# zerohd4869/MM-DFN

Hardware: AMD Instinct MI355X
Metric: utterances/sec (fwd+bwd), IEMOCAP-shaped batch (higher is better)
Workload: dtype f32; 1 GPU; cfg2 (BASELINE configs[1]): B=16 dialogues/GPU, L=110, dims 100/100/512, 2 GCN layers, P=2, dropout 0.50; utterances_per_gpu=1760, parallelism=dp1

## Files before the change

### include/mmdfn_hip.h

```cpp
#ifndef MMDFN_HIP_H
#define MMDFN_HIP_H

#include <stdint.h>

#ifdef __cplusplus
extern "C" {
#endif

int64_t mmdfn_riders_bytes(void);

int mmdfn_abi_version(void);

int mmdfn_propagate(const float* tiles, const float* cross, const float* H, float* out,
                    const int32_t* dia_len, const int32_t* row_start, const int64_t* tile_base,
                    int B, int M, int N, int d, int ldh, int ldo, int max_len, int transpose,
                    void* stream);

int mmdfn_tile_outer(const float* X, const float* Y, float* dtiles, float* dcross,
                     const int32_t* dia_len, const int32_t* row_start, const int64_t* tile_base,
                     int B, int M, int N, int d, int ldx, int ldy, int max_len, int accumulate,
                     void* stream);

int mmdfn_adj_build(const float* feats, float* unit, float* norm, float* cosg, float* cdot,
                    float* rdeg, float* tiles, float* cross,
// ... 52 lines not shown
int mmdfn_keep_flags_stage(float* out, int64_t n, float keep, void* state, void* riders, void* stream);
int mmdfn_keep_flags_flush(void* riders, void* stream);
int mmdfn_gru_seq_fwd_takes_flags(int ngroups, const int* rows);
int64_t mmdfn_colsum_workspace(int H);
int mmdfn_colsum(const float* A, int64_t R, int H, int lda, float* out, float* workspace, void* stream);
int mmdfn_colsum_partial(const float* A, int64_t R, int H, int lda, float* workspace, void* stream);
int mmdfn_party_combine(int Mn, const float* const* base, const float* E, const int32_t* rank,
                        const int64_t* flat_idx, float* out, const float* weights,
                        int L, int B, int P, int N, int H, void* stream);
int mmdfn_party_combine_bwd(int Mn, const float* dout, const int32_t* rank, const int64_t* flat_idx,
                            float* const* dbase, float* dE, const float* weights,
                            int L, int B, int P, int N, int H, void* stream);
int mmdfn_party_combine_bwd_dst(int Mn, const float* dout, const int32_t* rank, const int64_t* inv, float* const* dbase,
                                float* dE, const float* weights, int L, int B, int P, int N, int H, void* stream);


int mmdfn_mask_scale(int ngroups, const float* const* x, const float* const* mask, float* const* out,
                     const int64_t* n, float scale, void* stream);

int mmdfn_linear(const float* X, const float* W, const float* bias, float* Y, int R, int K, int N,
                 int ldx, int ldy, int act, int accumulate, void* stream);
int mmdfn_linear2(const float* X, const float* W, const float* W2, int N1, const float* bias, const float* bias2,
                  float* Y, int R, int K, int N, int ldx, int ldy, int act, int accumulate, void* stream);

int64_t mmdfn_weight_planes_workspace(int N, int K);
int mmdfn_cut_weight_planes(int n, const float* const* w1, const float* const* w2, const int* n1, const int* ld,
                            const int* N, const int* K, const int* mode, void* const* planes, void* stream);
int mmdfn_linear_planes(const float* X, const void* planes, const float* bias, const float* bias2, int n1, float* Y, int R,
                        int K, int N, int ldx, int ldy, int act, int accumulate, void* stream);
int mmdfn_linear_planes_group(int n, const float* const* X, const void* const* planes, const float* const* bias,
                              const float* const* bias2, const int* n1, float* const* Y, const int* R, const int* K,
                              const int* N, const int* ldx, const int* ldy, int act, int accumulate,
                              const float* const* mask, float mask_scale, void* stream);

int mmdfn_linear_group_supported(int R, int K, int N);
int mmdfn_linear_group(int n, const float* const* X, const float* const* W, const float* const* W2, const int* N1,
                       const float* const* bias, const float* const* bias2, float* const* Y, const int* R,
                       const int* K, const int* N, const int* ldx, const int* ldw, const int* ldy,
                       const int* kmajor, const int* accumulate, int act, void* stream);
int mmdfn_linear_group_addend(int n, const float* const* X, const float* const* W, const float* const* W2, const int* N1,
                              const float* const* bias, const float* const* bias2, float* const* Y, const float* const* Z,
                              const int* ldz, const int* R, const int* K, const int* N, const int* ldx, const int* ldw,
                              const int* ldy, const int* kmajor, const int* accumulate, int act, void* stream);

int mmdfn_softmax_scale_fwd(const float* z, const float* c, float* att, float* out, int R, int W, void* stream);
int mmdfn_softmax_scale_bwd(const float* att, const float* c, const float* dout, float* dz, float* dc, int R, int W,
                            void* stream);
int mmdfn_mfn_mem_fwd(const float* u, const float* v1, const float* v2, const float* mem, float* out, float* saved,
                      int64_t n, void* stream);
int mmdfn_mfn_mem_bwd(const float* saved, const float* mem, const float* dout, float* du, float* dv1, float* dv2,
                      float* dmem, int64_t n, void* stream);
int mmdfn_gated_pair_fwd(const float* xm, const float* xn, const float* w, const float* b, const float* pm,
                         const float* pn, float* out, float* zs, int R, int D, int C, void* stream);
int mmdfn_gated_pair_bwd(const float* xm, const float* xn, const float* w, const float* pm, const float* pn,
                         const float* zs, const float* dout, float* dxm, float* dxn, float* dpm, float* dpn,
                         float* dpre, int R, int D, int C, void* stream);
int mmdfn_rowscale_colsum(const float* s, const float* xm, const float* xn, float* out, int R, int D, void* stream);

int mmdfn_gemm_tn_splits(int R, int M, int N);
int mmdfn_gemm_tn(const float* A, const float* B, float* C, float* colsum, float* workspace,
                  int R, int M, int N, int lda, int ldb, int ldc, int splits, void* stream);

int64_t mmdfn_gemm_tn_grouped_workspace(int n, const int* R, const int* M, const int* N);
int mmdfn_gemm_tn_grouped(int n, const float* const* A, const float* const* B, float* const* C, float* const* colsum,
                          const int* R, const int* M, const int* N, const int* lda, const int* ldb, const int* ldc,
                          const int* bshift, float* workspace, void* stream);
// ... 87 lines not shown
```

### mm_dfn_amd/_hip.py

```python
import ctypes
import os

import torch

from . import build as _build

_P = ctypes.c_void_p
_I = ctypes.c_int
_F = ctypes.c_float
_L = ctypes.c_int64

SIGNATURES = {
    "mmdfn_abi_version": [],
    "mmdfn_propagate": [_P, _P, _P, _P, _P, _P, _P, _I, _I, _I, _I, _I, _I, _I, _I, _P],
    "mmdfn_tile_outer": [_P, _P, _P, _P, _P, _P, _P, _I, _I, _I, _I, _I, _I, _I, _I, _P],
    "mmdfn_adj_build": [_P] * 8 + [_P, _P, _P] + [_I] * 5 + [_F, _P],
    "mmdfn_adj_build_bwd": [_P] * 16 + [_P, _P, _P] + [_I] * 5 + [_F, _P],
    "mmdfn_riders_bytes": [],
    "mmdfn_gru_seq_fwd": [_I, _P, _P, _P, _P, _P, _P, _P, _I, _P, _P],
    "mmdfn_gru_seq_bwd": [_I, _P, _P, _P, _P, _P, _P, _P, _P, _I, _P, _P],
    "mmdfn_gru_seq_fwd_seg": [_I, _P, _P, _P, _P, _P, _P, _P, _I, _P, _P, _P, _P, _P, _P],
    "mmdfn_gru_seq_bwd_seg": [_I, _P, _P, _P, _P, _P, _P, _P, _P, _I, _P, _P, _P, _P, _P, _P, _P],
    "mmdfn_gru_tab_reduce": [_P, _P, _P, _P, _I, _I, _I, _I, _P],
    "mmdfn_lstm_pointwise_fwd": [_P, _P, _P, _P, _L, _I, _P],
    "mmdfn_lstm_pointwise_bwd": [_P, _P, _P, _P, _P, _P, _P, _L, _I, _P],
    "mmdfn_gcnii_combine_fwd": [_P, _P, _P, _P, _P, _F, _F, _L, _I, _P],
    "mmdfn_gcnii_combine_bwd": [_P, _P, _P, _P, _P, _P, _F, _F, _L, _I, _P],
    "mmdfn_gcn_input_fwd": [_P] * 8 + [_I] * 4 + [_F, _P],
    "mmdfn_gcn_input_bwd": [_P] * 9 + [_I] * 4 + [_F, _P],
    "mmdfn_lstm_gate_fwd": [_P] * 10 + [_I] * 2 + [_P],
    "mmdfn_lstm_gate_fwd_ld": [_P] * 10 + [_I] * 3 + [_P],
    "mmdfn_lstm_gate_fwd_pre": [_P] * 10 + [_I] * 3 + [_P, _P],
    "mmdfn_lstm_gate_planes_workspace": [_I],
    "mmdfn_lstm_gate_cut_weights": [_P, _P, _P, _I, _P],
    "mmdfn_lstm_gate_takes_planes": [_I, _I],
    "mmdfn_lstm_gate_bwd": [_P] * 13 + [_I] * 4 + [_P],
    "mmdfn_gcnii_layer_fwd": [_P] * 7 + [_F, _F, _I, _I, _I, _F, _P],
    "mmdfn_prop_layer_fwd": [_P, _P, _P, _I, _P, _P, _P, _I, _I, _I, _I, _P, _P, _P, _P, _P, _P, _P, _F, _F, _I, _I, _F, _P],
    "mmdfn_gcnii_layer_bwd": [_P] * 6 + [_F, _F, _I, _I, _I, _I, _P],
    "mmdfn_gcnii_layer_bwd_ld": [_P] * 6 + [_F, _F, _I, _I, _I, _I, _I, _P],
    "mmdfn_linear": [_P, _P, _P, _P, _I, _I, _I, _I, _I, _I, _I, _P],
    "mmdfn_linear2": [_P, _P, _P, _I, _P, _P, _P, _I, _I, _I, _I, _I, _I, _I, _P],
    "mmdfn_weight_planes_workspace": [_I, _I],
    "mmdfn_cut_weight_planes": [_I, _P, _P, _P, _P, _P, _P, _P, _P, _P],
    "mmdfn_linear_planes": [_P, _P, _P, _P, _I, _P, _I, _I, _I, _I, _I, _I, _I, _P],
    "mmdfn_linear_planes_group": [_I, _P, _P, _P, _P, _P, _P, _P, _P, _P, _P, _P, _I, _I, _P, _F, _P],
    "mmdfn_linear_group_supported": [_I, _I, _I],
    "mmdfn_linear_group": [_I] + [_P] * 15 + [_I, _P],
    "mmdfn_linear_group_addend": [_I] + [_P] * 17 + [_I, _P],
    "mmdfn_softmax_scale_fwd": [_P, _P, _P, _P, _I, _I, _P],
    "mmdfn_softmax_scale_bwd": [_P, _P, _P, _P, _P, _I, _I, _P],
    "mmdfn_mfn_mem_fwd": [_P] * 6 + [_L, _P],
    "mmdfn_mfn_mem_bwd": [_P] * 7 + [_L, _P],
    "mmdfn_gated_pair_fwd": [_P] * 8 + [_I, _I, _I, _P],
    "mmdfn_gated_pair_bwd": [_P] * 12 + [_I, _I, _I, _P],
    "mmdfn_rowscale_colsum": [_P, _P, _P, _P, _I, _I, _P],
    "mmdfn_gemm_tn_splits": [_I, _I, _I],
    "mmdfn_gemm_tn": [_P, _P, _P, _P, _P, _I, _I, _I, _I, _I, _I, _I, _P],
    "mmdfn_gemm_tn_grouped_workspace": [_I, _P, _P, _P],
    "mmdfn_gemm_tn_grouped": [_I, _P, _P, _P, _P, _P, _P, _P, _P, _P, _P, _P, _P, _P],
    "mmdfn_gemm_tn_batch_workspace": [_I, _P, _P, _I, _P, _P],
    "mmdfn_gemm_tn_batch": [_I, _P, _P, _P, _P, _P, _P, _P, _I, _P, _P, _P, _P, _P, _P, _P, _P, _P, _P],
    "mmdfn_wgrad_riders_stage": [_I, _P, _P, _P, _P, _P, _P, _P, _I, _P, _P, _P, _P, _P, _P, _P, _P, _P, _P],
    "mmdfn_wgrad_riders_staged": [_P],
    "mmdfn_wgrad_riders_flush": [_P, _P],
    "mmdfn_wgrad_riders_drain": [_P, _P, _I],
    "mmdfn_gru_seq_bwd_idle_cus": [_I, _P],
    "mmdfn_gru_seq_bwd_step_ns": [_I, _P],
    "mmdfn_gemm_tn_batch_ext": [_I, _P, _P, _P, _P, _P, _P, _P, _I, _P, _P, _P, _P, _P, _P, _P, _P,
                                _I, _P, _P, _P, _P, _P, _P, _P, _P, _P, _P, _P],
    "mmdfn_head_bwd_groups": [],
    "mmdfn_head_bwd_partial": [_P, _P, _P, _P, _P, _P, _P, _L, _I, _I, _I, _I, _I, _F, _P],
    "mmdfn_colsum_partial": [_P, _L, _I, _I, _P, _P],
    "mmdfn_head_fwd": [_P, _P, _P, _P, _P, _L, _I, _I, _I, _I, _F, _P],
    "mmdfn_head_bwd_workspace": [_I, _I],
    "mmdfn_head_bwd": [_P] * 9 + [_L, _I, _I, _I, _I, _I, _F, _P],
    "mmdfn_focal_loss_fwd": [_P, _P, _P, _P, _P, _L, _I, _F, _I, _P],
    "mmdfn_focal_loss_bwd": [_P, _P, _P, _P, _L, _I, _P],
    "mmdfn_focal_loss_fwd_grad": [_P, _P, _P, _P, _P, _P, _L, _I, _F, _I, _P],
    "mmdfn_focal_loss_fwd_ignore": [_P, _P, _P, _P, _P, _P, _L, _I, _F, _I, _L, _P],
    "mmdfn_focal_loss_bwd_ignore": [_P, _P, _P, _P, _P, _L, _I, _L, _P],
    "mmdfn_adam_step": [_P, _P, _P, _P, _L, _F, _F, _F, _F, _F, _I, _P],
    "mmdfn_party_gather": [_I, _P, _P, _P, _P, _P, _I, _I, _I, _I, _P],
    "mmdfn_party_gather_bwd": [_I, _P, _P, _P, _P, _I, _I, _I, _I, _P],
    "mmdfn_party_gather_bwd_colsum": [_I, _P, _P, _P, _P, _I, _I, _I, _I, _P, _P],
    "mmdfn_party_combine": [_I, _P, _P, _P, _P, _P, _P, _I, _I, _I, _I, _I, _P],
    "mmdfn_party_combine_bwd": [_I, _P, _P, _P, _P, _P, _P, _I, _I, _I, _I, _I, _P],
    "mmdfn_party_combine_bwd_dst": [_I, _P, _P, _P, _P, _P, _P, _I, _I, _I, _I, _I, _P],
    "mmdfn_mask_scale": [_I, _P, _P, _P, _P, _F, _P],
    "mmdfn_keep_flags": [_P, _L, _F, _P, _P],
    "mmdfn_keep_flags_stage": [_P, _L, _F, _P, _P, _P],
    "mmdfn_keep_flags_flush": [_P, _P],
    "mmdfn_gru_seq_fwd_takes_flags": [_I, _P],
    "mmdfn_colsum_workspace": [_I],
    "mmdfn_colsum": [_P, _L, _I, _I, _P, _P, _P],
}

ABI_VERSION = 18


class HipLibraryError(RuntimeError):
    pass


_libs = {}
_tuning = os.environ.get("MMDFN_TUNING_LIB", "0") == "1"


def set_tuning(flag):
    global _tuning
    prev, _tuning = _tuning, bool(flag)
    return prev


def lib():
    handle = _libs.get(_tuning)
    if handle is not None:
        return handle
    tuning = _tuning
    path = _build.TUNING_LIBPATH if tuning else _build.LIBPATH
    if _build.is_stale(tuning):
        try:
            _build.build(verbose=False, tuning=tuning)
        except Exception as e:
            raise HipLibraryError(
                "%s is missing or stale (source digest mismatch) and could not be rebuilt (%s): run `python -m "
                "mm_dfn_amd.build` (needs hipcc); the MI355X path has no CPU fallback" % (path, e)) from e
    handle = ctypes.CDLL(path)
    for name, argtypes in SIGNATURES.items():
        try:
            fn = getattr(handle, name)
# ... 57 lines not shown
```

### mm_dfn_amd/csrc/linear_planes.hip

```cpp
#include "planes_common.h"
#include "../../include/mmdfn_hip.h"

namespace {

constexpr int PL_MAXW = 16;

struct CutTable {
    const float* w1[PL_MAXW];
    const float* w2[PL_MAXW];
    u32x4* planes[PL_MAXW];
    int n1[PL_MAXW], ld[PL_MAXW];
    int N[PL_MAXW], K[PL_MAXW];
    int mode[PL_MAXW];
    int prefix[PL_MAXW + 1];
    int n;
};

__device__ __forceinline__ float cut_element(const CutTable& T, int i, int n, int k) {
    const int N = T.N[i], K = T.K[i], ld = T.ld[i], n1 = T.n1[i];
    if (n >= N || k >= K) return 0.f;
    int row, col;
    const float* base;
    switch (T.mode[i]) {
        case 0:
// ... 26 lines not shown
    const int g = blockIdx.x * 256 + threadIdx.x;
    if (g >= T.prefix[T.n]) return;
    int i = 0;
    while (i + 1 < T.n && g >= T.prefix[i + 1]) ++i;
    const int t = g - T.prefix[i];
    const int N = T.N[i], K = T.K[i], ld = T.ld[i], n1 = T.n1[i];
    const int KS = (K + 15) >> 4;
    const int lane = t & 63;
    const int f = t >> 6;
    const int ct = f / KS, ks = f - ct * KS;
    const int n = 32 * ct + (lane & 31);
    const int k0 = 16 * ks + 8 * (lane >> 5);
    float x[8];
    if (T.mode[i] == 0 && n < N && k0 + 8 <= K && (ld & 3) == 0) {
        const float* rp = (n < n1) ? T.w1[i] + (int64_t)n * ld + k0 : T.w2[i] + (int64_t)(n - n1) * ld + k0;
        const float4 a = *reinterpret_cast<const float4*>(rp), b = *reinterpret_cast<const float4*>(rp + 4);
        x[0] = a.x; x[1] = a.y; x[2] = a.z; x[3] = a.w; x[4] = b.x; x[5] = b.y; x[6] = b.z; x[7] = b.w;
    } else {
#pragma unroll
        for (int j = 0; j < 8; ++j) x[j] = cut_element(T, i, n, k0 + j);
    }
    u32x4 p1, p2, p3;
    pl_cut8(x, p1, p2, p3);
    u32x4* dst = T.planes[i] + (int64_t)f * 3 * 64 + lane;
    dst[0] = p1;
    dst[64] = p2;
    dst[128] = p3;
}

template <int RH>
__device__ __forceinline__ void linear_planes_body(
    u32x4* As, const float* __restrict__ X, const u32x4* __restrict__ planes, const float* __restrict__ bias,
    const float* __restrict__ bias2, int n1, float* __restrict__ Y, int R, int K, int N, int ldx, int ldy, int act,
    int accumulate, int nrb, int ncb, int bid, const float* __restrict__ mask = nullptr, float mscale = 1.0f) {
    constexpr int TPW = 4 / (3 - RH);
    constexpr int NACC = (RH == 2) ? 1 : 2;
    int rb, cb;
    if (!pl_decode(nrb, ncb, rb, cb, bid)) return;
    const int tid = threadIdx.x;
    const int lane = tid & 63;
    const int w = tid >> 6;
    const int KS = (K + 15) >> 4;
    const int NPH = (KS + PL_STG - 1) / PL_STG;
    const int NT = (N + 31) >> 5;
    const int ct = TPW * cb + (RH == 2 ? w : (w >> 1));
    const int myh = (RH == 2) ? 0 : (w & 1);
    const bool has_tile = ct < NT;
    const int r0 = rb * PL_BM;

    f32x16 acc[RH][NACC];
#pragma unroll
    for (int h = 0; h < RH; ++h)
#pragma unroll
        for (int c = 0; c < NACC; ++c)
#pragma unroll
            for (int r = 0; r < 16; ++r) acc[h][c][r] = 0.f;

    const u32x4* bsrc = planes + ((int64_t)(has_tile ? ct : 0) * KS) * 3 * 64 + lane;
    f32x4 raw[2][2];
    const int shf = w & 1, sksl = w >> 1;
    const int srow = r0 + 32 * shf + (lane & 31);
    const float* xrow = X + (int64_t)(srow < R ? srow : R - 1) * ldx;
    const int skofs = 16 * sksl + 8 * (lane >> 5);

#define PL_ISSUE_X(PAR, PH)                                                                                 \
    do {                                                                                                    \
        const int k0_ = 16 * PL_STG * (PH) + skofs;                                                         \
        raw[PAR][0] = *reinterpret_cast<const f32x4*>(xrow + (k0_ < K ? k0_ : 0));                          \
        raw[PAR][1] = *reinterpret_cast<const f32x4*>(xrow + (k0_ + 4 < K ? k0_ + 4 : 0));                  \
    } while (0)
#define PL_PARK(PAR, PH, BUF)                                                                               \
    do {                                                                                                    \
        const int k0_ = 16 * PL_STG * (PH) + skofs;                                                         \
        const bool ok0_ = k0_ < K, ok1_ = k0_ + 4 < K;        \
        float x_[8] = {ok0_ ? raw[PAR][0].x : 0.f, ok0_ ? raw[PAR][0].y : 0.f, ok0_ ? raw[PAR][0].z : 0.f, ok0_ ? raw[PAR][0].w : 0.f, \
                       ok1_ ? raw[PAR][1].x : 0.f, ok1_ ? raw[PAR][1].y : 0.f, ok1_ ? raw[PAR][1].z : 0.f, ok1_ ? raw[PAR][1].w : 0.f}; \
        u32x4 p1_, p2_, p3_;                                                                                \
        pl_cut8(x_, p1_, p2_, p3_);                                                                         \
        u32x4* dst_ = &As[(BUF) * (PL_LDS / 2) + ((sksl * 3) * 2 + shf) * 64 + lane];                       \
        dst_[0] = p1_;                                                                                      \
        dst_[2 * 64] = p2_;                                                                                 \
        dst_[4 * 64] = p3_;                                                                                 \
    } while (0)
#include "planes_pipeline.h"
#undef PL_PARK
#undef PL_ISSUE_X

    if (!has_tile) return;
    const int col = 32 * ct + (lane & 31);
    if (col >= N) return;
    float bv = 0.f;
    if (col < n1) { if (bias) bv = bias[col]; }
    else if (bias2) bv = bias2[col - n1];
    float mv[RH][16];
#pragma unroll
    for (int h = 0; h < RH; ++h)
#pragma unroll
        for (int r = 0; r < 16; ++r) {
            const int row = r0 + 32 * (RH == 2 ? h : myh) + (r & 3) + 8 * (r >> 2) + 4 * (lane >> 5);
            mv[h][r] = 1.0f;
            if (mask) mv[h][r] = mask[(int64_t)(row < R ? row : R - 1) * N + col] * mscale;
        }
#pragma unroll
    for (int h = 0; h < RH; ++h)
#pragma unroll
        for (int r = 0; r < 16; ++r) {
            const int row = r0 + 32 * (RH == 2 ? h : myh) + (r & 3) + 8 * (r >> 2) + 4 * (lane >> 5);
            if (row < R) {
                float* yp = Y + (int64_t)row * ldy + col;
                float v = (NACC == 2 ? acc[h][0][r] + acc[h][NACC - 1][r] : acc[h][0][r]) + bv;
                if (act == 1) v = v > 0.f ? v : 0.f;
                v *= mv[h][r];
                if (accumulate) v += *yp;
                *yp = v;
            }
        }
}

template <int RH>
__global__ __launch_bounds__(256, 4) void linear_planes_kernel(
    const float* __restrict__ X, const u32x4* __restrict__ planes, const float* __restrict__ bias,
    const float* __restrict__ bias2, int n1, float* __restrict__ Y, int R, int K, int N, int ldx, int ldy, int act,
    int accumulate, int nrb, int ncb) {
    __shared__ u32x4 As[PL_LDS];
    linear_planes_body<RH>(As, X, planes, bias, bias2, n1, Y, R, K, N, ldx, ldy, act, accumulate, nrb, ncb, (int)blockIdx.x);
}

constexpr int PL_MAXG = 4;
struct PlGroup {
    const float* X[PL_MAXG];
    const u32x4* planes[PL_MAXG];
    const float* bias[PL_MAXG];
    const float* bias2[PL_MAXG];
    float* Y[PL_MAXG];
    const float* mask[PL_MAXG];
    int n1[PL_MAXG], R[PL_MAXG], K[PL_MAXG], N[PL_MAXG], ldx[PL_MAXG], ldy[PL_MAXG], nrb[PL_MAXG], ncb[PL_MAXG], rh[PL_MAXG];
    int blk0[PL_MAXG + 1];
    int n;
};

__global__ __launch_bounds__(256, 4) void linear_planes_group_kernel(PlGroup G, int act, int accumulate, float mscale) {
    __shared__ u32x4 As[PL_LDS];
    int p = 0;
    while (p + 1 < G.n && (int)blockIdx.x >= G.blk0[p + 1]) ++p;
    const int bid = (int)blockIdx.x - G.blk0[p];
    if (G.rh[p] == 2)
        linear_planes_body<2>(As, G.X[p], G.planes[p], G.bias[p], G.bias2[p], G.n1[p], G.Y[p], G.R[p], G.K[p], G.N[p], G.ldx[p],
                              G.ldy[p], act, accumulate, G.nrb[p], G.ncb[p], bid, G.mask[p], mscale);
    else
        linear_planes_body<1>(As, G.X[p], G.planes[p], G.bias[p], G.bias2[p], G.n1[p], G.Y[p], G.R[p], G.K[p], G.N[p], G.ldx[p],
                              G.ldy[p], act, accumulate, G.nrb[p], G.ncb[p], bid, G.mask[p], mscale);
}

inline void pl_form(int R, int N, int* nrb, int* ncb, int* rh) {
    *nrb = (R + PL_BM - 1) / PL_BM;
    const int NT = (N + 31) / 32;
    const bool narrow = (int64_t)*nrb * ((NT + 3) / 4) < 400;
    *ncb = narrow ? (NT + 1) / 2 : (NT + 3) / 4;
    *rh = narrow ? 1 : 2;
}

}

extern "C" {

int64_t mmdfn_weight_planes_workspace(int N, int K) {
    if (N <= 0 || K <= 0) return -1;
    const int64_t NT = (N + 31) / 32, KS = (K + 15) / 16;
    return NT * KS * 3 * 64 * 16;
}

int mmdfn_cut_weight_planes(int n, const float* const* w1, const float* const* w2, const int* n1, const int* ld,
                            const int* N, const int* K, const int* mode, void* const* planes, void* stream) {
    if (n <= 0 || n > PL_MAXW) return -1;
    CutTable T;
    T.n = n;
    T.prefix[0] = 0;
    for (int i = 0; i < n; ++i) {
        if (!w1[i] || !planes[i] || N[i] <= 0 || K[i] <= 0 || mode[i] < 0 || mode[i] > 3) return -1;
        if ((reinterpret_cast<uintptr_t>(planes[i]) & 15) != 0) return -1;
        if ((ld[i] & 3) == 0 && ((reinterpret_cast<uintptr_t>(w1[i]) & 15) || (w2[i] && (reinterpret_cast<uintptr_t>(w2[i]) & 15))))
            return -1;
        const int split_extent = mode[i] == 0 ? N[i] : mode[i] == 1 ? K[i] : N[i];
        if (n1[i] < split_extent && !w2[i]) return -1;
        if (mode[i] == 3 && (K[i] & 3)) return -1;
        T.w1[i] = w1[i];
        T.w2[i] = w2[i];
        T.planes[i] = reinterpret_cast<u32x4*>(planes[i]);
        T.n1[i] = n1[i];
        T.ld[i] = ld[i];
        T.N[i] = N[i];
        T.K[i] = K[i];
        T.mode[i] = mode[i];
        const int64_t tasks = (int64_t)((N[i] + 31) / 32) * ((K[i] + 15) / 16) * 64;
        if (T.prefix[i] + tasks > (1ll << 30)) return -1;
        T.prefix[i + 1] = T.prefix[i] + (int)tasks;
    }
    hipLaunchKernelGGL(cut_planes_kernel, dim3((T.prefix[n] + 255) / 256), dim3(256), 0, (hipStream_t)stream, T);
    MMDFN_CHECK_LAUNCH();
    return 0;
}

int mmdfn_linear_planes(const float* X, const void* planes, const float* bias, const float* bias2, int n1, float* Y, int R,
                        int K, int N, int ldx, int ldy, int act, int accumulate, void* stream) {
    if (R <= 0) return 0;
    if (!X || !planes || !Y || K < 4 || (K & 3) || N <= 0 || (ldx & 3) || ldx < K || ldy < N) return -1;
    if ((reinterpret_cast<uintptr_t>(X) & 15) || (reinterpret_cast<uintptr_t>(planes) & 15)) return -1;
    int nrb, ncb, rh;
    pl_form(R, N, &nrb, &ncb, &rh);
    const bool narrow = rh == 1;
    const int64_t grid = pl_grid(nrb, ncb);
    if (grid > (1ll << 30)) return -1;
    if (narrow)
        hipLaunchKernelGGL(linear_planes_kernel<1>, dim3((unsigned)grid), dim3(256), 0, (hipStream_t)stream, X,
                           reinterpret_cast<const u32x4*>(planes), bias, bias2, n1, Y, R, K, N, ldx, ldy, act, accumulate, nrb, ncb);
    else
        hipLaunchKernelGGL(linear_planes_kernel<2>, dim3((unsigned)grid), dim3(256), 0, (hipStream_t)stream, X,
                           reinterpret_cast<const u32x4*>(planes), bias, bias2, n1, Y, R, K, N, ldx, ldy, act, accumulate, nrb, ncb);
    MMDFN_CHECK_LAUNCH();
    return 0;
}

int mmdfn_linear_planes_group(int n, const float* const* X, const void* const* planes, const float* const* bias,
                              const float* const* bias2, const int* n1, float* const* Y, const int* R, const int* K,
                              const int* N, const int* ldx, const int* ldy, int act, int accumulate,
                              const float* const* mask, float mask_scale, void* stream) {
    if (n <= 0 || n > PL_MAXG) return -1;
    PlGroup G;
    G.n = 0;
    G.blk0[0] = 0;
    for (int i = 0; i < n; ++i) {
        if (R[i] <= 0) continue;
        if (!X[i] || !planes[i] || !Y[i] || K[i] < 4 || (K[i] & 3) || N[i] <= 0 || (ldx[i] & 3) || ldx[i] < K[i] || ldy[i] < N[i])
            return -1;
        if ((reinterpret_cast<uintptr_t>(X[i]) & 15) || (reinterpret_cast<uintptr_t>(planes[i]) & 15)) return -1;
        const int p = G.n++;
        G.X[p] = X[i];
        G.planes[p] = reinterpret_cast<const u32x4*>(planes[i]);
        G.bias[p] = bias ? bias[i] : nullptr;
        G.bias2[p] = bias2 ? bias2[i] : nullptr;
        G.Y[p] = Y[i];
        G.mask[p] = mask ? mask[i] : nullptr;
        G.n1[p] = n1[i]; G.R[p] = R[i]; G.K[p] = K[i]; G.N[p] = N[i]; G.ldx[p] = ldx[i]; G.ldy[p] = ldy[i];
        pl_form(R[i], N[i], &G.nrb[p], &G.ncb[p], &G.rh[p]);
        const int64_t blocks = pl_grid(G.nrb[p], G.ncb[p]);
        if (G.blk0[p] + blocks > (1ll << 30)) return -1;
        G.blk0[p + 1] = G.blk0[p] + (int)blocks;
    }
    if (G.n == 0) return 0;
    for (int p = G.n; p < PL_MAXG; ++p) {
        G.X[p] = nullptr; G.planes[p] = nullptr; G.bias[p] = G.bias2[p] = nullptr; G.Y[p] = nullptr; G.mask[p] = nullptr;
        G.n1[p] = G.R[p] = G.K[p] = G.N[p] = G.ldx[p] = G.ldy[p] = G.nrb[p] = G.ncb[p] = G.rh[p] = 0;
        G.blk0[p + 1] = G.blk0[G.n];
    }
    hipLaunchKernelGGL(linear_planes_group_kernel, dim3((unsigned)G.blk0[G.n]), dim3(256), 0, (hipStream_t)stream, G, act,
                       accumulate, mask_scale);
    MMDFN_CHECK_LAUNCH();
    return 0;
}

}
```

### mm_dfn_amd/csrc/planes_common.h

```cpp
#pragma once
#include "mmdfn_internal.h"

namespace {

typedef __bf16 pl_bf16x8 __attribute__((ext_vector_type(8)));
typedef uint32_t u32x4 __attribute__((ext_vector_type(4)));
typedef uint32_t u32x2 __attribute__((ext_vector_type(2)));
typedef float f32x16 __attribute__((ext_vector_type(16)));

constexpr int PL_BM = 64;
constexpr int PL_STG = 2;
constexpr int PL_LDS = 2 * PL_STG * 3 * 2 * 64;

__device__ __forceinline__ float pl_as_f(uint32_t u) { return __builtin_bit_cast(float, u); }
__device__ __forceinline__ uint32_t pl_as_u(float f) { return __builtin_bit_cast(uint32_t, f); }
__device__ __forceinline__ f32x16 pl_mfma(u32x4 a, u32x4 b, f32x16 c) {
    return __builtin_amdgcn_mfma_f32_32x32x16_bf16(__builtin_bit_cast(pl_bf16x8, a), __builtin_bit_cast(pl_bf16x8, b), c, 0, 0, 0);
}

__device__ __forceinline__ void pl_cut2(float a, float b, uint32_t& p1, uint32_t& p2, uint32_t& p3) {
    p1 = __builtin_amdgcn_perm(pl_as_u(b), pl_as_u(a), 0x07060302u);
    a -= pl_as_f(pl_as_u(a) & 0xffff0000u);
    b -= pl_as_f(pl_as_u(b) & 0xffff0000u);
    p2 = __builtin_amdgcn_perm(pl_as_u(b), pl_as_u(a), 0x07060302u);
    a -= pl_as_f(pl_as_u(a) & 0xffff0000u);
    b -= pl_as_f(pl_as_u(b) & 0xffff0000u);
    p3 = __builtin_amdgcn_perm(pl_as_u(b), pl_as_u(a), 0x07060302u);
}
__device__ __forceinline__ void pl_cut8(const float (&x)[8], u32x4& p1, u32x4& p2, u32x4& p3) {
#pragma unroll
    for (int j = 0; j < 4; ++j) {
        uint32_t q1, q2, q3;
        pl_cut2(x[2 * j], x[2 * j + 1], q1, q2, q3);
        p1[j] = q1;
        p2[j] = q2;
        p3[j] = q3;
    }
}

__device__ __forceinline__ bool pl_decode(int nrb, int ncb, int& rb, int& cb, int bid) {
    const int yq = bid >> 3;
    rb = (yq / ncb) * 8 + (bid & 7);
    cb = yq % ncb;
    return rb < nrb;
}
inline int64_t pl_grid(int nrb, int ncb) { return (int64_t)((nrb + 7) / 8) * 8 * ncb; }

}
```

### mm_dfn_amd/csrc/propagate.hip

```cpp
#include "mmdfn_internal.h"
#include "../../include/mmdfn_hip.h"
#include <stdlib.h>

namespace {

constexpr int BK = 32;

template <int NW, int NCT, bool TRANS>
__global__ __launch_bounds__(64 * NW) void propagate_kernel(
    const float* __restrict__ tiles, const float* __restrict__ cross, const float* __restrict__ H,
    float* __restrict__ out, const int32_t* __restrict__ dia_len, const int32_t* __restrict__ row_start,
    const int64_t* __restrict__ tile_base, int M, int N, int d, int ldh, int ldo, int max_rb) {
    constexpr int BM = 16 * NW;
    constexpr int CB = 16 * NCT;
    constexpr int LDH = CB + 2;
    constexpr int LDT = BM + 2;
    __shared__ float Hs[BK * LDH];
    __shared__ float Ts[TRANS ? BK * LDT : 1];

    const int i = blockIdx.x / max_rb;
    const int rb = blockIdx.x % max_rb;
    const int m = blockIdx.y;
    const int c0 = blockIdx.z * CB;
    const int L = dia_len[i];
// ... 370 lines not shown
            case 5: return V2(4, 2, 4, 16, 1);
            case 6: return V2(4, 1, 7, 16, 2);
            case 7: return V2(4, 2, 7, 16, 1);
            case 8: {
                const int rc = mmdfn_launch_propagate_split(tiles, cross, H, out, dia_len, row_start, tile_base, B, M, N, d,
                                                            ldh, ldo, max_len, s);
                if (rc != -2) return rc;
                break;
            }
            default: break;
        }
    }
    if (ov == 9) {
        if (d <= 112) return ((long)B * M * max_len <= 32768L) ? V2(2, 4, 2, 16, 1) : V2(8, 1, 7, 16, 1);
        if (d <= 224) return V2(4, 2, 7, 16, 1);
        return V2(4, 2, 4, 16, 1);
    }
    const long approx_rows = (long)B * M * max_len;
    const long split_wgs = (long)B * M * ((max_len + 127) / 128) * ((d + 127) / 128);
    if (max_len >= 128 && split_wgs >= 48) {
        const int rc = mmdfn_launch_propagate_split(tiles, cross, H, out, dia_len, row_start, tile_base, B, M, N, d, ldh,
                                                    ldo, max_len, s);
        if (rc != -2) return rc;
    }
    if (d <= 112) {
        if (approx_rows <= 32768L) return V2(2, 4, 2, 16, 1);
        return V2(8, 1, 7, 16, 1);
    }
    if (d <= 224) return V2(4, 2, 7, 16, 1);
    return V2(4, 2, 4, 16, 1);
}
#undef V2

extern "C" int mmdfn_abi_version(void) { return 18; }

extern "C" int mmdfn_propagate(const float* tiles, const float* cross, const float* H, float* out,
                               const int32_t* dia_len, const int32_t* row_start, const int64_t* tile_base,
                               int B, int M, int N, int d, int ldh, int ldo, int max_len, int transpose,
                               void* stream) {
    return mmdfn_launch_propagate(tiles, cross, H, out, dia_len, row_start, tile_base, B, M, N, d, ldh, ldo, max_len,
                                  transpose, (hipStream_t)stream);
}
```

### mm_dfn_amd/ops_linear.py

```python
import torch

from . import _hip
from .ops_pad import pad4, row_operand, weight_operand
from .ops_wgrad import _queueable, _wgrad, _wgrad_inline, queue_wgrad


def linear_raw(x2d, weight, bias=None, act=0, out=None, accumulate=False):
    _hip.require_cuda(x2d, weight)
    _hip.require_f32(x2d, weight, bias, out)
    R, K = x2d.shape
    N = weight.shape[0]
    if x2d.stride(1) != 1 or x2d.stride(0) % 4 or x2d.data_ptr() % 16:
        x2d = x2d.contiguous()
    weight = weight.contiguous()
    if out is None:
        out = torch.empty(R, N, dtype=torch.float32, device=x2d.device)
    rc = _hip.lib().mmdfn_linear(_hip.ptr(x2d), _hip.ptr(weight), _hip.ptr(bias), _hip.ptr(out), R, K, N,
                                 x2d.stride(0), out.stride(0), int(act), 1 if accumulate else 0, _hip.stream())
    _hip.check(rc, "mmdfn_linear")
    return out


def linear_group_raw(problems, act=0):
    n = len(problems)
# ... 419 lines not shown
    _PLANE_EPOCH[0] += 1


class planes_recording:

    def __enter__(self):
        self.used = []
        _PLANE_RECORDERS.append(self.used)
        return self.used

    def __exit__(self, *exc):
        _PLANE_RECORDERS.remove(self.used)
        return False


def linear_planes_raw(x2, w1, w2=None, b1=None, b2=None, transposed=False, act=0, out=None, accumulate=False):
    _hip.require_cuda(x2, w1)
    _hip.require_f32(x2, w1, w2, b1, b2, out)
    if x2.stride(1) != 1 or x2.stride(0) % 4 or x2.data_ptr() % 16:
        x2 = x2.contiguous()
    e = weight_planes(w1, w2, transposed)
    R, K = x2.shape
    if K != e.K:
        raise ValueError("linear_planes_raw: contraction width %d, planes were cut for %d" % (K, e.K))
    if out is None:
        out = torch.empty(R, e.N, dtype=torch.float32, device=x2.device)
    n1 = e.N if (transposed or w2 is None) else e.n1
    rc = _hip.lib().mmdfn_linear_planes(_hip.ptr(x2), _hip.ptr(e.buf), _hip.ptr(b1), _hip.ptr(b2), n1, _hip.ptr(out), R, K, e.N,
                                        x2.stride(0), out.stride(0), int(act), 1 if accumulate else 0, _hip.stream())
    _hip.check(rc, "mmdfn_linear_planes")
    return out


def linear_planes_group_raw(problems, transposed=False, act=0, mask_scale=1.0):
    lib = _hip.lib()
    xs, ents, outs = [], [], []
    for pr in problems:
        x2 = pr["x"]
        _hip.require_cuda(x2, pr["w1"])
        _hip.require_f32(x2, pr["w1"], pr.get("w2"), pr.get("b1"), pr.get("b2"), pr.get("out"))
        if x2.stride(1) != 1 or x2.stride(0) % 4 or x2.data_ptr() % 16:
            x2 = x2.contiguous()
        e = weight_planes(pr["w1"], pr.get("w2"), transposed)
        if x2.shape[1] != e.K:
            raise ValueError("linear_planes_group_raw: contraction width %d, planes were cut for %d" % (x2.shape[1], e.K))
        out = pr.get("out")
        if out is None:
            out = torch.empty(x2.shape[0], e.N, dtype=torch.float32, device=x2.device)
        mk = pr.get("mask")
        if mk is not None and (mk.numel() != out.numel() or mk.dtype != torch.float32 or not mk.is_contiguous() or out.stride(0) != e.N):
            raise _hip.HipLibraryError("linear_planes_group_raw: mask must be contiguous fp32 flags of the (contiguous) output's size")
        xs.append(x2)
        ents.append(e)
        outs.append(out)
    for i in range(0, len(problems), 4):
        sl = slice(i, i + 4)
        prs, x4, e4, o4 = problems[sl], xs[sl], ents[sl], outs[sl]
        n1 = [e.N if (transposed or pr.get("w2") is None) else e.n1 for pr, e in zip(prs, e4)]
        rc = lib.mmdfn_linear_planes_group(len(prs), _hip.ptr_array(x4), _hip.ptr_array([e.buf for e in e4]),
                                           _hip.ptr_array([pr.get("b1") for pr in prs]), _hip.ptr_array([pr.get("b2") for pr in prs]),
                                           _hip.int_array(n1), _hip.ptr_array(o4), _hip.int_array([x.shape[0] for x in x4]),
                                           _hip.int_array([e.K for e in e4]), _hip.int_array([e.N for e in e4]),
                                           _hip.int_array([x.stride(0) for x in x4]), _hip.int_array([o.stride(0) for o in o4]),
                                           int(act), 0, _hip.ptr_array([pr.get("mask") for pr in prs]), float(mask_scale),
                                           _hip.stream())
        _hip.check(rc, "mmdfn_linear_planes_group")
    return outs


class _Linear2Group(torch.autograd.Function):

    @staticmethod
    def forward(ctx, n, masks, scale, *args):
        grp = [args[5 * g:5 * g + 5] for g in range(n)]
        shapes, x2s = [], []
        if masks is not None:
            from .ops_flags import _MaskScale
            xin = [x.contiguous() for x, *_ in grp]
            dropped = [torch.empty_like(x) for x in xin]
            _MaskScale._launch(xin, list(masks), dropped, float(scale))
        for g, (x, w1, w2, b1, b2) in enumerate(grp):
            shapes.append(x.shape)
            x2 = (dropped[g] if masks is not None else x).reshape(-1, x.shape[-1])
            if x2.stride(1) != 1 or x2.stride(0) % 4 or x2.data_ptr() % 16:
                x2 = x2.contiguous()
            x2s.append(x2)
        ys = linear_planes_group_raw([dict(x=x2, w1=w1, w2=w2, b1=b1, b2=b2) for x2, (_, w1, w2, b1, b2) in zip(x2s, grp)])
        ctx.n = n
        ctx.masks = None if masks is None else list(masks)
        ctx.scale = float(scale)
        ctx.refs = [(w1, w2, b1, b2) for _, w1, w2, b1, b2 in grp]
        ctx.save_for_backward(*x2s)
        return tuple(y.view(*shp[:-1], y.shape[1]) for y, shp in zip(ys, shapes))

    @staticmethod
    def backward(ctx, *dys):
        x2s = ctx.saved_tensors
        n = ctx.n
        dy2s = []
        for g in range(n):
            dy = dys[g]
            if dy is None:
                N = ctx.refs[g][0].shape[0] + ctx.refs[g][1].shape[0]
                dy = torch.zeros(x2s[g].shape[0], N, dtype=torch.float32, device=x2s[g].device)
            dy2s.append(dy.reshape(-1, dy.shape[-1]).contiguous())
        need = [g for g in range(n) if ctx.needs_input_grad[3 + 5 * g]]
        dxs = [None] * n
        if need:
            got = linear_planes_group_raw([dict(x=dy2s[g], w1=ctx.refs[g][0], w2=ctx.refs[g][1],
                                                mask=None if ctx.masks is None else ctx.masks[g]) for g in need],
                                          transposed=True, mask_scale=ctx.scale)
            for g, dx in zip(need, got):
                dxs[g] = dx
        out = [None, None, None]
        for g in range(n):
            p1, p2, b1, b2 = ctx.refs[g]
            n1 = p1.shape[0]
            d1, d2 = dy2s[g][:, :n1], dy2s[g][:, n1:]
            dw1, db1 = _wgrad(d1, x2s[g], p1, b1)
            dw2, db2 = _wgrad(d2, x2s[g], p2, b2)
            dx = dxs[g]
            if dx is not None:
                lead = dys[g].shape[:-1] if dys[g] is not None else (x2s[g].shape[0],)
                dx = dx.view(*lead, p1.shape[1])
            out += [dx, dw1, dw2, db1, db2]
        return tuple(out)


def linear2_group(groups, masks=None, scale=1.0):
    rows = sum(int(x.numel() // x.shape[-1]) for x, *_ in groups)
    if (len(groups) >= 2 and rows >= PLANES_MIN_ROWS and all(x.is_cuda and x.dtype == torch.float32 for x, *_ in groups)
            and all(planes_supported(w1, w2) and b1 is not None and b2 is not None for _, w1, w2, b1, b2 in groups)
            and (masks is None or all(m.numel() == x.numel() and x.numel() % 4 == 0 for m, (x, *_) in zip(masks, groups)))):
        flat = [t for grp in groups for t in grp]
        return list(_Linear2Group.apply(len(groups), None if masks is None else list(masks), float(scale), *flat))
    return None


LINEAR2_FEW_ROWS = 2048
GROUP_ROWS = 4096


def linear2(x, w1, w2, b1, b2, wcat=None, bcat=None):
    if w1.shape[1] % 4 or w1.shape[1] < 4:
# ... 13 lines not shown
```

Baseline: 2.146 million utterances/s.

## Add split-K path to grouped planes linear for backward dX GEMM

Adds a split-K variant of the grouped planes linear kernel. Each K slice writes fp32 partials to a workspace, and a second reduce kernel sums them and applies bias, activation, mask and accumulate. The backward input-gradient call in _Linear2Group now asks for automatic split selection, which picks split 2 when K is large and the grid is small, to fill more CUs. The cost is an extra kernel launch, a workspace allocation and extra partial-sum memory traffic.

```diff
diff --git a/include/mmdfn_hip.h b/include/mmdfn_hip.h
--- a/include/mmdfn_hip.h
+++ b/include/mmdfn_hip.h
@@ -108,6 +108,11 @@
                               const float* const* bias2, const int* n1, float* const* Y, const int* R, const int* K,
                               const int* N, const int* ldx, const int* ldy, int act, int accumulate,
                               const float* const* mask, float mask_scale, void* stream);
+int64_t mmdfn_linear_planes_group_workspace(int n, const int* R, const int* K, const int* N, int split);
+int mmdfn_linear_planes_group_split(int n, const float* const* X, const void* const* planes, const float* const* bias,
+                                    const float* const* bias2, const int* n1, float* const* Y, const int* R, const int* K,
+                                    const int* N, const int* ldx, const int* ldy, int act, int accumulate,
+                                    const float* const* mask, float mask_scale, int split, float* workspace, void* stream);
 
 int mmdfn_linear_group_supported(int R, int K, int N);
 int mmdfn_linear_group(int n, const float* const* X, const float* const* W, const float* const* W2, const int* N1,
diff --git a/mm_dfn_amd/_hip.py b/mm_dfn_amd/_hip.py
--- a/mm_dfn_amd/_hip.py
+++ b/mm_dfn_amd/_hip.py
@@ -45,6 +45,8 @@
     "mmdfn_cut_weight_planes": [_I, _P, _P, _P, _P, _P, _P, _P, _P, _P],
     "mmdfn_linear_planes": [_P, _P, _P, _P, _I, _P, _I, _I, _I, _I, _I, _I, _I, _P],
     "mmdfn_linear_planes_group": [_I, _P, _P, _P, _P, _P, _P, _P, _P, _P, _P, _P, _I, _I, _P, _F, _P],
+    "mmdfn_linear_planes_group_workspace": [_I, _P, _P, _P, _I],
+    "mmdfn_linear_planes_group_split": [_I, _P, _P, _P, _P, _P, _P, _P, _P, _P, _P, _P, _I, _I, _P, _F, _I, _P, _P],
     "mmdfn_linear_group_supported": [_I, _I, _I],
     "mmdfn_linear_group": [_I] + [_P] * 15 + [_I, _P],
     "mmdfn_linear_group_addend": [_I] + [_P] * 17 + [_I, _P],
@@ -96,7 +98,7 @@
     "mmdfn_colsum": [_P, _L, _I, _I, _P, _P, _P],
 }
 
-ABI_VERSION = 18
+ABI_VERSION = 19
 
 
 class HipLibraryError(RuntimeError):
diff --git a/mm_dfn_amd/csrc/linear_planes.hip b/mm_dfn_amd/csrc/linear_planes.hip
--- a/mm_dfn_amd/csrc/linear_planes.hip
+++ b/mm_dfn_amd/csrc/linear_planes.hip
@@ -82,7 +82,8 @@
 __device__ __forceinline__ void linear_planes_body(
     u32x4* As, const float* __restrict__ X, const u32x4* __restrict__ planes, const float* __restrict__ bias,
     const float* __restrict__ bias2, int n1, float* __restrict__ Y, int R, int K, int N, int ldx, int ldy, int act,
-    int accumulate, int nrb, int ncb, int bid, const float* __restrict__ mask = nullptr, float mscale = 1.0f) {
+    int accumulate, int nrb, int ncb, int bid, const float* __restrict__ mask = nullptr, float mscale = 1.0f,
+    int kbeg = 0, int kend = 0, float* __restrict__ part = nullptr) {
     constexpr int TPW = 4 / (3 - RH);
     constexpr int NACC = (RH == 2) ? 1 : 2;
     int rb, cb;
@@ -90,7 +91,8 @@
     const int tid = threadIdx.x;
     const int lane = tid & 63;
     const int w = tid >> 6;
-    const int KS = (K + 15) >> 4;
+    const int KL = (part ? kend : K) - kbeg;
+    const int KS = (KL + 15) >> 4;
     const int NPH = (KS + PL_STG - 1) / PL_STG;
     const int NT = (N + 31) >> 5;
     const int ct = TPW * cb + (RH == 2 ? w : (w >> 1));
@@ -106,23 +108,23 @@
 #pragma unroll
             for (int r = 0; r < 16; ++r) acc[h][c][r] = 0.f;
 
-    const u32x4* bsrc = planes + ((int64_t)(has_tile ? ct : 0) * KS) * 3 * 64 + lane;
+    const u32x4* bsrc = planes + ((int64_t)(has_tile ? ct : 0) * ((K + 15) >> 4) + (kbeg >> 4)) * 3 * 64 + lane;
     f32x4 raw[2][2];
     const int shf = w & 1, sksl = w >> 1;
     const int srow = r0 + 32 * shf + (lane & 31);
-    const float* xrow = X + (int64_t)(srow < R ? srow : R - 1) * ldx;
+    const float* xrow = X + (int64_t)(srow < R ? srow : R - 1) * ldx + kbeg;
     const int skofs = 16 * sksl + 8 * (lane >> 5);
 
 #define PL_ISSUE_X(PAR, PH)                                                                                 \
     do {                                                                                                    \
         const int k0_ = 16 * PL_STG * (PH) + skofs;                                                         \
-        raw[PAR][0] = *reinterpret_cast<const f32x4*>(xrow + (k0_ < K ? k0_ : 0));                          \
-        raw[PAR][1] = *reinterpret_cast<const f32x4*>(xrow + (k0_ + 4 < K ? k0_ + 4 : 0));                  \
+        raw[PAR][0] = *reinterpret_cast<const f32x4*>(xrow + (k0_ < KL ? k0_ : 0));                         \
+        raw[PAR][1] = *reinterpret_cast<const f32x4*>(xrow + (k0_ + 4 < KL ? k0_ + 4 : 0));                 \
     } while (0)
 #define PL_PARK(PAR, PH, BUF)                                                                               \
     do {                                                                                                    \
         const int k0_ = 16 * PL_STG * (PH) + skofs;                                                         \
-        const bool ok0_ = k0_ < K, ok1_ = k0_ + 4 < K;        \
+        const bool ok0_ = k0_ < KL, ok1_ = k0_ + 4 < KL;      \
         float x_[8] = {ok0_ ? raw[PAR][0].x : 0.f, ok0_ ? raw[PAR][0].y : 0.f, ok0_ ? raw[PAR][0].z : 0.f, ok0_ ? raw[PAR][0].w : 0.f, \
                        ok1_ ? raw[PAR][1].x : 0.f, ok1_ ? raw[PAR][1].y : 0.f, ok1_ ? raw[PAR][1].z : 0.f, ok1_ ? raw[PAR][1].w : 0.f}; \
         u32x4 p1_, p2_, p3_;                                                                                \
@@ -139,6 +141,16 @@
     if (!has_tile) return;
     const int col = 32 * ct + (lane & 31);
     if (col >= N) return;
+    if (part) {
+#pragma unroll
+        for (int h = 0; h < RH; ++h)
+#pragma unroll
+            for (int r = 0; r < 16; ++r) {
+                const int row = r0 + 32 * (RH == 2 ? h : myh) + (r & 3) + 8 * (r >> 2) + 4 * (lane >> 5);
+                if (row < R) part[(int64_t)row * N + col] = NACC == 2 ? acc[h][0][r] + acc[h][NACC - 1][r] : acc[h][0][r];
+            }
+        return;
+    }
     float bv = 0.f;
     if (col < n1) { if (bias) bv = bias[col]; }
     else if (bias2) bv = bias2[col - n1];
@@ -184,7 +196,9 @@
     const float* bias2[PL_MAXG];
     float* Y[PL_MAXG];
     const float* mask[PL_MAXG];
+    float* part[PL_MAXG];
     int n1[PL_MAXG], R[PL_MAXG], K[PL_MAXG], N[PL_MAXG], ldx[PL_MAXG], ldy[PL_MAXG], nrb[PL_MAXG], ncb[PL_MAXG], rh[PL_MAXG];
+    int split[PL_MAXG], kper[PL_MAXG];
     int blk0[PL_MAXG + 1];
     int n;
 };
@@ -193,13 +207,73 @@
     __shared__ u32x4 As[PL_LDS];
     int p = 0;
     while (p + 1 < G.n && (int)blockIdx.x >= G.blk0[p + 1]) ++p;
-    const int bid = (int)blockIdx.x - G.blk0[p];
+    int bid = (int)blockIdx.x - G.blk0[p];
+    const int g1 = (int)pl_grid(G.nrb[p], G.ncb[p]);
+    const int sl = bid / g1;
+    bid -= sl * g1;
+    const int kbeg = sl * G.kper[p];
+    const int kend = min(G.K[p], kbeg + G.kper[p]);
+    float* part = G.split[p] > 1 ? G.part[p] + (int64_t)sl * G.R[p] * G.N[p] : nullptr;
     if (G.rh[p] == 2)
         linear_planes_body<2>(As, G.X[p], G.planes[p], G.bias[p], G.bias2[p], G.n1[p], G.Y[p], G.R[p], G.K[p], G.N[p], G.ldx[p],
-                              G.ldy[p], act, accumulate, G.nrb[p], G.ncb[p], bid, G.mask[p], mscale);
+                              G.ldy[p], act, accumulate, G.nrb[p], G.ncb[p], bid, G.mask[p], mscale, kbeg, kend, part);
     else
         linear_planes_body<1>(As, G.X[p], G.planes[p], G.bias[p], G.bias2[p], G.n1[p], G.Y[p], G.R[p], G.K[p], G.N[p], G.ldx[p],
-                              G.ldy[p], act, accumulate, G.nrb[p], G.ncb[p], bid, G.mask[p], mscale);
+                              G.ldy[p], act, accumulate, G.nrb[p], G.ncb[p], bid, G.mask[p], mscale, kbeg, kend, part);
+}
+
+constexpr int PL_RROWS = 16;
+struct PlReduce {
+    const float* part[PL_MAXG];
+    const float* bias[PL_MAXG];
+    const float* bias2[PL_MAXG];
+    float* Y[PL_MAXG];
+    const float* mask[PL_MAXG];
+    int n1[PL_MAXG], R[PL_MAXG], N[PL_MAXG], ldy[PL_MAXG], split[PL_MAXG];
+    int blk0[PL_MAXG + 1];
+    int n;
+};
+
+__global__ __launch_bounds__(256) void linear_planes_reduce_kernel(PlReduce G, int act, int accumulate, float mscale) {
+    int p = 0;
+    while (p + 1 < G.n && (int)blockIdx.x >= G.blk0[p + 1]) ++p;
+    const int b = (int)blockIdx.x - G.blk0[p];
+    constexpr int RQ = PL_BM / PL_RROWS;
+    const int yq = b >> 3;
+    const int rb = (yq / RQ) * 8 + (b & 7);
+    const int row0 = rb * PL_BM + (yq % RQ) * PL_RROWS;
+    const int R = G.R[p], N = G.N[p], n1 = G.n1[p], split = G.split[p];
+    if (row0 >= R) return;
+    const int nq = N >> 2;
+    const int cnt = min(PL_RROWS, R - row0) * nq;
+    const int64_t slab = (int64_t)R * N;
+    const float* bias = G.bias[p];
+    const float* bias2 = G.bias2[p];
+    const float* mask = G.mask[p];
+    for (int i = threadIdx.x; i < cnt; i += 256) {
+        const int row = row0 + i / nq, col = 4 * (i % nq);
+        const int64_t o = (int64_t)row * N + col;
+        f32x4 v = *reinterpret_cast<const f32x4*>(G.part[p] + o);
+        for (int s = 1; s < split; ++s) v += *reinterpret_cast<const f32x4*>(G.part[p] + s * slab + o);
+        f32x4 m = {1.f, 1.f, 1.f, 1.f};
+        if (mask) m = *reinterpret_cast<const f32x4*>(mask + o) * mscale;
+        float* yp = G.Y[p] + (int64_t)row * G.ldy[p] + col;
+        f32x4 y;
+        if (accumulate) y = *reinterpret_cast<const f32x4*>(yp);
+#pragma unroll
+        for (int j = 0; j < 4; ++j) {
+            const int c = col + j;
+            float bv = 0.f;
+            if (c < n1) { if (bias) bv = bias[c]; }
+            else if (bias2) bv = bias2[c - n1];
+            float t = v[j] + bv;
+            if (act == 1) t = t > 0.f ? t : 0.f;
+            t *= m[j];
+            if (accumulate) t += y[j];
+            v[j] = t;
+        }
+        *reinterpret_cast<f32x4*>(yp) = v;
+    }
 }
 
 inline void pl_form(int R, int N, int* nrb, int* ncb, int* rh) {
@@ -208,6 +282,25 @@
     const bool narrow = (int64_t)*nrb * ((NT + 3) / 4) < 400;
     *ncb = narrow ? (NT + 1) / 2 : (NT + 3) / 4;
     *rh = narrow ? 1 : 2;
+}
+
+inline int pl_split(int K, int N, int nrb, int* ncb, int* rh, int want, int* kper) {
+    const int nph = (K + 16 * PL_STG - 1) / (16 * PL_STG);
+    const int wide = ((N + 31) / 32 + 3) / 4;
+    int s = 1;
+    if (want > 0) s = want;
+    else if (K >= 400 && pl_grid(nrb, wide) < 2 * 256) s = 2;
+    if (N % 4 || s < 1) s = 1;
+    if (s > 4) s = 4;
+    if (s > nph) s = nph;
+    const int pps = (nph + s - 1) / s;
+    s = (nph + pps - 1) / pps;
+    *kper = s > 1 ? 16 * PL_STG * pps : K;
+    if (s > 1) {
+        *ncb = wide;
+        *rh = 2;
+    }
+    return s;
 }
 
 }
@@ -271,12 +364,31 @@
     return 0;
 }
 
-int mmdfn_linear_planes_group(int n, const float* const* X, const void* const* planes, const float* const* bias,
-                              const float* const* bias2, const int* n1, float* const* Y, const int* R, const int* K,
-                              const int* N, const int* ldx, const int* ldy, int act, int accumulate,
-                              const float* const* mask, float mask_scale, void* stream) {
-    if (n <= 0 || n > PL_MAXG) return -1;
+int64_t mmdfn_linear_planes_group_workspace(int n, const int* R, const int* K, const int* N, int split) {
+    if (n <= 0 || n > PL_MAXG || split < 0) return -1;
+    int64_t floats = 0;
+    for (int i = 0; i < n; ++i) {
+        if (R[i] <= 0) continue;
+        if (K[i] < 4 || N[i] <= 0) return -1;
+        int nrb, ncb, rh, kper;
+        pl_form(R[i], N[i], &nrb, &ncb, &rh);
+        const int s = pl_split(K[i], N[i], nrb, &ncb, &rh, split, &kper);
+        if (s > 1) floats += (int64_t)s * R[i] * N[i];
+    }
+    return floats;
+}
+
+int mmdfn_linear_planes_group_split(int n, const float* const* X, const void* const* planes, const float* const* bias,
+                                    const float* const* bias2, const int* n1, float* const* Y, const int* R, const int* K,
+                                    const int* N, const int* ldx, const int* ldy, int act, int accumulate,
+                                    const float* const* mask, float mask_scale, int split, float* workspace, void* stream) {
+    if (n <= 0 || n > PL_MAXG || split < 0) return -1;
+    if (reinterpret_cast<uintptr_t>(workspace) & 15) return -1;
     PlGroup G;
+    PlReduce Q;
+    Q.n = 0;
+    Q.blk0[0] = 0;
+    float* ws = workspace;
     G.n = 0;
     G.blk0[0] = 0;
     for (int i = 0; i < n; ++i) {
@@ -293,20 +405,56 @@
         G.mask[p] = mask ? mask[i] : nullptr;
         G.n1[p] = n1[i]; G.R[p] = R[i]; G.K[p] = K[i]; G.N[p] = N[i]; G.ldx[p] = ldx[i]; G.ldy[p] = ldy[i];
         pl_form(R[i], N[i], &G.nrb[p], &G.ncb[p], &G.rh[p]);
-        const int64_t blocks = pl_grid(G.nrb[p], G.ncb[p]);
+        G.split[p] = pl_split(K[i], N[i], G.nrb[p], &G.ncb[p], &G.rh[p], split, &G.kper[p]);
+        if (G.split[p] > 1 &&
+            ((ldy[i] & 3) || (reinterpret_cast<uintptr_t>(Y[i]) & 15) || (G.mask[p] && (reinterpret_cast<uintptr_t>(G.mask[p]) & 15)))) {
+            pl_form(R[i], N[i], &G.nrb[p], &G.ncb[p], &G.rh[p]);
+            G.split[p] = 1;
+            G.kper[p] = K[i];
+        }
+        G.part[p] = nullptr;
+        if (G.split[p] > 1) {
+            if (!ws) return -1;
+            G.part[p] = ws;
+            ws += (int64_t)G.split[p] * R[i] * N[i];
+            const int q = Q.n++;
+            Q.part[q] = G.part[p]; Q.bias[q] = G.bias[p]; Q.bias2[q] = G.bias2[p]; Q.Y[q] = G.Y[p]; Q.mask[q] = G.mask[p];
+            Q.n1[q] = n1[i]; Q.R[q] = R[i]; Q.N[q] = N[i]; Q.ldy[q] = ldy[i]; Q.split[q] = G.split[p];
+            Q.blk0[q + 1] = Q.blk0[q] + (int)(pl_grid(G.nrb[p], 1) * (PL_BM / PL_RROWS));
+        }
+        const int64_t blocks = pl_grid(G.nrb[p], G.ncb[p]) * G.split[p];
         if (G.blk0[p] + blocks > (1ll << 30)) return -1;
         G.blk0[p + 1] = G.blk0[p] + (int)blocks;
     }
     if (G.n == 0) return 0;
     for (int p = G.n; p < PL_MAXG; ++p) {
         G.X[p] = nullptr; G.planes[p] = nullptr; G.bias[p] = G.bias2[p] = nullptr; G.Y[p] = nullptr; G.mask[p] = nullptr;
-        G.n1[p] = G.R[p] = G.K[p] = G.N[p] = G.ldx[p] = G.ldy[p] = G.nrb[p] = G.ncb[p] = G.rh[p] = 0;
+        G.part[p] = nullptr;
+        G.n1[p] = G.R[p] = G.K[p] = G.N[p] = G.ldx[p] = G.ldy[p] = G.nrb[p] = G.ncb[p] = G.rh[p] = G.kper[p] = 0;
+        G.split[p] = 1;
         G.blk0[p + 1] = G.blk0[G.n];
     }
     hipLaunchKernelGGL(linear_planes_group_kernel, dim3((unsigned)G.blk0[G.n]), dim3(256), 0, (hipStream_t)stream, G, act,
                        accumulate, mask_scale);
     MMDFN_CHECK_LAUNCH();
+    if (Q.n == 0) return 0;
+    for (int q = Q.n; q < PL_MAXG; ++q) {
+        Q.part[q] = nullptr; Q.bias[q] = Q.bias2[q] = nullptr; Q.Y[q] = nullptr; Q.mask[q] = nullptr;
+        Q.n1[q] = Q.R[q] = Q.N[q] = Q.ldy[q] = Q.split[q] = 0;
+        Q.blk0[q + 1] = Q.blk0[Q.n];
+    }
+    hipLaunchKernelGGL(linear_planes_reduce_kernel, dim3((unsigned)Q.blk0[Q.n]), dim3(256), 0, (hipStream_t)stream, Q, act, accumulate,
+                       mask_scale);
+    MMDFN_CHECK_LAUNCH();
     return 0;
 }
 
-}
+int mmdfn_linear_planes_group(int n, const float* const* X, const void* const* planes, const float* const* bias,
+                              const float* const* bias2, const int* n1, float* const* Y, const int* R, const int* K,
+                              const int* N, const int* ldx, const int* ldy, int act, int accumulate,
+                              const float* const* mask, float mask_scale, void* stream) {
+    return mmdfn_linear_planes_group_split(n, X, planes, bias, bias2, n1, Y, R, K, N, ldx, ldy, act, accumulate, mask, mask_scale,
+                                           1, nullptr, stream);
+}
+
+}
diff --git a/mm_dfn_amd/csrc/planes_common.h b/mm_dfn_amd/csrc/planes_common.h
--- a/mm_dfn_amd/csrc/planes_common.h
+++ b/mm_dfn_amd/csrc/planes_common.h
@@ -44,6 +44,6 @@
     cb = yq % ncb;
     return rb < nrb;
 }
-inline int64_t pl_grid(int nrb, int ncb) { return (int64_t)((nrb + 7) / 8) * 8 * ncb; }
+__host__ __device__ inline int64_t pl_grid(int nrb, int ncb) { return (int64_t)((nrb + 7) / 8) * 8 * ncb; }
 
 }
diff --git a/mm_dfn_amd/csrc/propagate.hip b/mm_dfn_amd/csrc/propagate.hip
--- a/mm_dfn_amd/csrc/propagate.hip
+++ b/mm_dfn_amd/csrc/propagate.hip
@@ -426,7 +426,7 @@
 }
 #undef V2
 
-extern "C" int mmdfn_abi_version(void) { return 18; }
+extern "C" int mmdfn_abi_version(void) { return 19; }
 
 extern "C" int mmdfn_propagate(const float* tiles, const float* cross, const float* H, float* out,
                                const int32_t* dia_len, const int32_t* row_start, const int64_t* tile_base,
diff --git a/mm_dfn_amd/ops_linear.py b/mm_dfn_amd/ops_linear.py
--- a/mm_dfn_amd/ops_linear.py
+++ b/mm_dfn_amd/ops_linear.py
@@ -475,7 +475,7 @@
     return out
 
 
-def linear_planes_group_raw(problems, transposed=False, act=0, mask_scale=1.0):
+def linear_planes_group_raw(problems, transposed=False, act=0, mask_scale=1.0, split=1):
     lib = _hip.lib()
     xs, ents, outs = [], [], []
     for pr in problems:
@@ -500,14 +500,18 @@
         sl = slice(i, i + 4)
         prs, x4, e4, o4 = problems[sl], xs[sl], ents[sl], outs[sl]
         n1 = [e.N if (transposed or pr.get("w2") is None) else e.n1 for pr, e in zip(prs, e4)]
-        rc = lib.mmdfn_linear_planes_group(len(prs), _hip.ptr_array(x4), _hip.ptr_array([e.buf for e in e4]),
+        rows, ks, ns = _hip.int_array([x.shape[0] for x in x4]), _hip.int_array([e.K for e in e4]), _hip.int_array([e.N for e in e4])
+        nws = lib.mmdfn_linear_planes_group_workspace(len(prs), rows, ks, ns, int(split))
+        if nws < 0:
+            raise _hip.HipLibraryError("mmdfn_linear_planes_group_workspace rejected the group")
+        ws = torch.empty(nws, dtype=torch.float32, device=x4[0].device) if nws > 0 else None
+        rc = lib.mmdfn_linear_planes_group_split(len(prs), _hip.ptr_array(x4), _hip.ptr_array([e.buf for e in e4]),
                                            _hip.ptr_array([pr.get("b1") for pr in prs]), _hip.ptr_array([pr.get("b2") for pr in prs]),
-                                           _hip.int_array(n1), _hip.ptr_array(o4), _hip.int_array([x.shape[0] for x in x4]),
-                                           _hip.int_array([e.K for e in e4]), _hip.int_array([e.N for e in e4]),
+                                           _hip.int_array(n1), _hip.ptr_array(o4), rows, ks, ns,
                                            _hip.int_array([x.stride(0) for x in x4]), _hip.int_array([o.stride(0) for o in o4]),
                                            int(act), 0, _hip.ptr_array([pr.get("mask") for pr in prs]), float(mask_scale),
-                                           _hip.stream())
-        _hip.check(rc, "mmdfn_linear_planes_group")
+                                           int(split), _hip.ptr(ws), _hip.stream())
+        _hip.check(rc, "mmdfn_linear_planes_group_split")
     return outs
 
 
@@ -552,7 +556,7 @@
         if need:
             got = linear_planes_group_raw([dict(x=dy2s[g], w1=ctx.refs[g][0], w2=ctx.refs[g][1],
                                                 mask=None if ctx.masks is None else ctx.masks[g]) for g in need],
-                                          transposed=True, mask_scale=ctx.scale)
+                                          transposed=True, mask_scale=ctx.scale, split=0)
             for g, dx in zip(need, got):
                 dxs[g] = dx
         out = [None, None, None]
```

Measured after the change: 2.151 million utterances/s, median of 6. No clear change (+0.2%).
